# dwofk/fast-depth

Hardware: AMD Instinct MI355X
Metric: frames/sec (224x224) MobileNet-NNConv5dw-skipadd inference forward (higher is better)
Workload: dtype f32; 1 GPU; configs[1]: MobileNet-NNConv5(dw)+skipadd unpruned, batch=32 per GPU, 224x224 fp32 inference forward, inputs resident in HBM; batch_per_gpu=32, global_batch=32, parallelism=frames sharded over 1 GPU(s), no collective, rccl_ranks=0, input_batches_in_rotation=8

## Files before the change

fast-depth_amd/csrc/fd_infer_launch.h:

```cpp
#pragma once
namespace {

template <typename T, int ACT>
int launch_stem(const Layer &L, const float *x, const float *wp, const float *bias, T *y, int B, hipStream_t s)
{
    switch (L.chunk) {
    case 32: FD_LAUNCH((fd_stem3x3s2<T, ACT, 32>), L.grid, dim3(256), L.lds, s, x, wp, bias, y, B, L.in_h, L.in_w, L.d.cout); break;
    case 16: FD_LAUNCH((fd_stem3x3s2<T, ACT, 16>), L.grid, dim3(256), L.lds, s, x, wp, bias, y, B, L.in_h, L.in_w, L.d.cout); break;
    default: FD_LAUNCH((fd_stem3x3s2<T, ACT, 8>), L.grid, dim3(256), L.lds, s, x, wp, bias, y, B, L.in_h, L.in_w, L.d.cout); break;
    }
    return check_launch("fd_stem3x3s2");
}

template <typename T, int K, int S, int MODE, int ACT>
int launch_dw_inst(const Layer &L, const T *in, const T *skip, const float *wp, const float *bias, T *out, hipStream_t s)
{
    if constexpr (!std::is_same<T, float>::value) {
        if (L.dw_n == 8) {
            FD_LAUNCH((fd_dwconv<T, K, S, MODE, ACT, 8>), L.grid, dim3(256), L.lds, s, in, skip, wp, bias, out,
                      L.in_h, L.in_w, L.out_h, L.out_w, L.d.cin, L.cbq, L.th, L.tw, L.tiles_x, L.csplit, L.pstr);
            return check_launch("fd_dwconv");
        }
    }
    FD_LAUNCH((fd_dwconv<T, K, S, MODE, ACT, 4>), L.grid, dim3(256), L.lds, s, in, skip, wp, bias, out,
                       L.in_h, L.in_w, L.out_h, L.out_w, L.d.cin, L.cbq, L.th, L.tw, L.tiles_x, L.csplit, L.pstr);
    return check_launch("fd_dwconv");
}

template <typename T, int ACT>
int launch_dw(const Layer &L, const T *in, const T *skip, const float *wp, const float *bias, T *out, hipStream_t s, const unsigned *wpk = nullptr)
{
    if (L.dw5_cl) {
        if constexpr (!std::is_same<T, float>::value) {
            if (L.dw5_cl == 64)
                FD_LAUNCH((fd_dw5_rows<T, ACT, 64>), L.grid, dim3(FD_DW5R_BLOCK), 0, s, in, skip, wpk, bias, out, L.in_h, L.in_w, L.d.cin, L.dw5_cbs, L.dw5_groups, L.dw5_bh);
            else
                FD_LAUNCH((fd_dw5_rows<T, ACT, 32>), L.grid, dim3(FD_DW5R_BLOCK), 0, s, in, skip, wpk, bias, out, L.in_h, L.in_w, L.d.cin, L.dw5_cbs, L.dw5_groups, L.dw5_bh);
            return check_launch("fd_dw5_rows");
        }
        return fail(FD_ERR_INVALID, "fd_dw5_rows is a 16-bit kernel");
    }
    if (L.dw_rows && L.dw_rows8) {
        if constexpr (!std::is_same<T, float>::value) {
            if (L.d.stride == 1)
                FD_LAUNCH((fd_dw3_rows8<T, 1, ACT>), L.grid, dim3(256), 0, s, in, wp, bias, out, L.in_h, L.in_w, L.out_h, L.out_w, L.d.cin, L.th);
            else
                FD_LAUNCH((fd_dw3_rows8<T, 2, ACT>), L.grid, dim3(256), 0, s, in, wp, bias, out, L.in_h, L.in_w, L.out_h, L.out_w, L.d.cin, L.th);
            return check_launch("fd_dw3_rows8");
        }
    }
    if (L.dw_rows) {
        if (L.d.stride == 1)
            FD_LAUNCH((fd_dw3_rows<T, 1, ACT>), L.grid, dim3(256), 0, s, in, wp, bias, out, L.in_h, L.in_w, L.out_h, L.out_w, L.d.cin, L.th);
        else
            FD_LAUNCH((fd_dw3_rows<T, 2, ACT>), L.grid, dim3(256), 0, s, in, wp, bias, out, L.in_h, L.in_w, L.out_h, L.out_w, L.d.cin, L.th);
        return check_launch("fd_dw3_rows");
    }
    const int key = L.d.ksize * 100 + L.d.stride * 10 + L.mode;
    switch (key) {
    case 310: return launch_dw_inst<T, 3, 1, 0, ACT>(L, in, skip, wp, bias, out, s);
    case 320: return launch_dw_inst<T, 3, 2, 0, ACT>(L, in, skip, wp, bias, out, s);
    case 510: return launch_dw_inst<T, 5, 1, 0, ACT>(L, in, skip, wp, bias, out, s);
    case 511: return launch_dw_inst<T, 5, 1, 1, ACT>(L, in, skip, wp, bias, out, s);
    case 512: return launch_dw_inst<T, 5, 1, 2, ACT>(L, in, skip, wp, bias, out, s);
    case 311: return launch_dw_inst<T, 3, 1, 1, ACT>(L, in, skip, wp, bias, out, s);
    case 312: return launch_dw_inst<T, 3, 1, 2, ACT>(L, in, skip, wp, bias, out, s);
    case 513: return launch_dw_inst<T, 5, 1, 3, ACT>(L, in, skip, wp, bias, out, s);
    }
    return fail(FD_ERR_INVALID, "depthwise k=%d stride=%d mode=%d has no kernel", L.d.ksize, L.d.stride, L.mode);
}

template <int ACT>
int launch_pw(const fd_plan *plan, const Layer &L, const float *A, const float *wp, const float *bias, float *out, long M, hipStream_t s)
{
    const int N = L.d.cout, K = L.d.cin;
    if (L.pw16_tm) {
        fd_dwfuse fz{};
        int fdw = 0;
        if (L.fuse_next_dw >= 0) {
            const Layer &D = plan->layers[L.fuse_next_dw];
            fz.w = reinterpret_cast<const float *>(plan->ws + D.w_off); fz.b = reinterpret_cast<const float *>(plan->ws + D.b_off);
            fz.out = reinterpret_cast<float *>(plan->ws + D.out_off);
            fz.H = L.out_h; fz.W = L.out_w; fz.S = D.d.stride; fz.up = D.d.upsample;
            fz.hi = D.d.act == FD_ACT_RELU6 ? 6.0f : __builtin_inff();
            fz.store_pw = (plan->flags & FD_PLAN_KEEP_ACTIVATIONS) ? 1 : 0;
            fdw = D.d.ksize;
        }
#define FD_PW16_LAUNCH(TMV, FD_) \
        do { (void)hipFuncSetAttribute((const void *)fd_pw_gemm16_f32<TMV, FD_G16_STAGES, ACT, 0, FD_>, hipFuncAttributeMaxDynamicSharedMemorySize, (int)L.lds); \
             FD_LAUNCH((fd_pw_gemm16_f32<TMV, FD_G16_STAGES, ACT, 0, FD_>), L.grid, dim3(512), L.lds, s, A, wp, bias, out, (int)M, N, K, L.w_pitch, L.pw16_stride, L.m_tiles, L.n_tiles, fz, fd_g16_train{}); } while (0)
#define FD_PW16_CASE(TMV) \
    case TMV: if (fdw == 3) FD_PW16_LAUNCH(TMV, 3); else if (fdw == 5) FD_PW16_LAUNCH(TMV, 5); else FD_PW16_LAUNCH(TMV, 0); break;
        switch (L.pw16_tm) {
            FD_PW16_CASE(13)
            FD_PW16_CASE(7)
            FD_PW16_CASE(4)
        default: return fail(FD_ERR_INVALID, "no gemm16 instance for TM=%d", L.pw16_tm);
        }
#undef FD_PW16_CASE
#undef FD_PW16_LAUNCH
        return check_launch("fd_pw_gemm16_f32");
    }
    const int key = L.pw.wgm * 1000 + L.pw.wgn * 100 + L.pw.tm * 10 + L.pw.tn;
#define FD_PW_CASE(a, b, c, d) \
    case a * 1000 + b * 100 + c * 10 + d: \
        if (L.lds > 64 * 1024) (void)hipFuncSetAttribute((const void *)fd_pw_gemm_f32<a, b, c, d, ACT>, hipFuncAttributeMaxDynamicSharedMemorySize, (int)L.lds); \
        FD_LAUNCH((fd_pw_gemm_f32<a, b, c, d, ACT>), L.grid, dim3(256), L.lds, s, A, wp, bias, out, (int)M, N, K, L.w_pitch, L.m_tiles, L.n_tiles); break;
    switch (key) {
        FD_PW_CASE(2, 2, 2, 2)
        FD_PW_CASE(2, 2, 2, 1)
        FD_PW_CASE(2, 2, 1, 2)
        FD_PW_CASE(2, 2, 1, 1)
        FD_PW_CASE(4, 1, 1, 1)
    default: return fail(FD_ERR_INVALID, "no pointwise tile %d", key);
    }
#undef FD_PW_CASE
    return check_launch("fd_pw_gemm_f32");
}



template <int ACT>
int launch_dwpw(const fd_plan *p, const Layer &L, float *out, float *y, hipStream_t s)
// ... 133 lines not shown
```

fast-depth_amd/csrc/fd_kernels_dw5p.h:

```cpp
#pragma once
#include "fd_device.h"

#ifdef FD_EMU
#define FD_INLINE_LAMBDA
#else
#define FD_INLINE_LAMBDA __attribute__((always_inline))
#endif

template <typename T>
__global__ void __launch_bounds__(256)
fd_pack_dw5_pairs(const float *__restrict__ wf, unsigned *__restrict__ wpk, int C)
{
    const int i = blockIdx.x * 256 + threadIdx.x;
    if (i >= 30 * C) return;
    const int c = i % C, q = i / C, ky = q / 6, k = q - ky * 6;
    const float *w = wf + (long)(ky * 5) * C + c;
    const float w0 = w[0], w1 = w[C], w2 = w[2 * C], w3 = w[3 * C], w4 = w[4 * C];
    float a, b;
    switch (k) {
    case 0: a = w0; b = w1; break;
    case 1: a = w2; b = w3; break;
    case 2: a = w4; b = 0.f; break;
    case 3: a = 0.f; b = w0; break;
    case 4: a = w1; b = w2; break;
// ... 92 lines not shown
    auto issue_a = [&](int it) FD_INLINE_LAMBDA {
        const int r = y0 - 2 + 2 * it;
        nv = r >= 0 && r < H;
        if (!nv) return;
        const unsigned ro = (unsigned)r * rowb;
#pragma unroll
        for (int p = 0; p < 4; ++p) { ns[0][2 * p] = fd_buf_ld32(r_skip, so[p], ro); ns[0][2 * p + 1] = fd_buf_ld32(r_skip, so[p], ro + pxb); }
    };
    auto issue_b = [&](int it) FD_INLINE_LAMBDA {
        const int r = y0 - 2 + 2 * it;
        nv_b = r >= 0 && r < H;
        if (!nv_b) return;
        const unsigned ro = (unsigned)(r + 1) * rowb, rl = (unsigned)(r >> 1) * (rowb >> 1);
#pragma unroll
        for (int p = 0; p < 4; ++p) { ns[1][2 * p] = fd_buf_ld32(r_skip, so[p], ro); ns[1][2 * p + 1] = fd_buf_ld32(r_skip, so[p], ro + pxb); nl[p] = fd_buf_ld32(r_low, lo_[p], rl); }
    };

    unsigned win[5][4][2];
#pragma unroll
    for (int a = 0; a < 5; ++a)
#pragma unroll
        for (int p = 0; p < 4; ++p) { win[a][p][0] = 0u; win[a][p][1] = 0u; }

    auto convert = [&](auto SLOT, const unsigned (&raw)[8], bool rv) FD_INLINE_LAMBDA {
        constexpr int slot = decltype(SLOT)::value;
        if (rv) fd_dw5_make_pairs(T{}, raw, nl, win[slot]);
        else {
#pragma unroll
            for (int p = 0; p < 4; ++p) { win[slot][p][0] = 0u; win[slot][p][1] = 0u; }
        }
    };
    auto out_row = [&](auto SB, int y) FD_INLINE_LAMBDA {
        constexpr int sb = decltype(SB)::value;
        float acc[4][2];
#pragma unroll
        for (int ky = 0; ky < 5; ++ky) {
            const unsigned (&R)[4][2] = win[(sb + ky) % 5];
#pragma unroll
            for (int k = 0; k < 3; ++k) {
#pragma unroll
                for (int ch = 0; ch < 2; ++ch) {
                    if (ky == 0 && k == 0) {
                        const float bb = ch ? b1 : b0;
                        acc[0][ch] = fd_dot2_first(T{}, R[k][ch], w[ky][k][ch], bb);
                        acc[1][ch] = fd_dot2_first(T{}, R[k][ch], w[ky][3 + k][ch], bb);
                        acc[2][ch] = fd_dot2_first(T{}, R[k + 1][ch], w[ky][k][ch], bb);
                        acc[3][ch] = fd_dot2_first(T{}, R[k + 1][ch], w[ky][3 + k][ch], bb);
                    } else {
                        fd_dot2_acc(T{}, R[k][ch], w[ky][k][ch], acc[0][ch]);
                        fd_dot2_acc(T{}, R[k][ch], w[ky][3 + k][ch], acc[1][ch]);
                        fd_dot2_acc(T{}, R[k + 1][ch], w[ky][k][ch], acc[2][ch]);
                        fd_dot2_acc(T{}, R[k + 1][ch], w[ky][3 + k][ch], acc[3][ch]);
                    }
                }
            }
        }
        fd_dot2_done(acc);
        if (y < y1) {
#pragma unroll
            for (int j = 0; j < 4; ++j) fd_buf_st32(r_out, oo, (unsigned)y * rowb + (unsigned)j * pxb, fd_dw5_pack_act<T, ACT>(acc[j][0], acc[j][1]));
        }
    };

    const int n_it = (y1 - y0 + 4) >> 1;
    issue_a(0); issue_b(0);
    auto step = [&](auto PH, int it) FD_INLINE_LAMBDA {
        constexpr int ph = decltype(PH)::value;
        const bool more = it + 1 < n_it;
        convert(fd_int<(2 * ph) % 5>{}, ns[0], nv);
        if (more) issue_a(it + 1);
        if (it >= 2) out_row(fd_int<(2 * ph + 1) % 5>{}, y0 - 4 + 2 * it);
        convert(fd_int<(2 * ph + 1) % 5>{}, ns[1], nv_b);
        if (more) issue_b(it + 1);
        if (it >= 2) out_row(fd_int<(2 * ph + 2) % 5>{}, y0 - 3 + 2 * it);
    };
    for (int it0 = 0; it0 < n_it; it0 += 5) {
        step(fd_int<0>{}, it0);
        if (it0 + 1 < n_it) step(fd_int<1>{}, it0 + 1);
        if (it0 + 2 < n_it) step(fd_int<2>{}, it0 + 2);
        if (it0 + 3 < n_it) step(fd_int<3>{}, it0 + 3);
        if (it0 + 4 < n_it) step(fd_int<4>{}, it0 + 4);
    }
}
```

fast-depth_amd/csrc/fd_plan_build.h:

```cpp
#pragma once
namespace {

int plan_layers(fd_plan *p, const fd_layer_desc *layers, size_t *woff_out)
{
    const size_t esz = p->dtype == FD_F32 ? 4 : 2;
    const int n_layers = (int)p->layers.size(), batch = p->B, height = p->H, width = p->W, dtype = p->dtype;
    const uint32_t flags = p->flags, tune = p->tune;
    (void)n_layers; (void)batch; (void)height; (void)width; (void)dtype; (void)flags; (void)tune;
    size_t woff = 0;
    for (int i = 0; i < n_layers; ++i) {
        Layer &L = p->layers[i];
        L.d = layers[i];
        const fd_layer_desc &d = L.d;
#define FD_BAD(...) do { return fail(FD_ERR_INVALID, __VA_ARGS__); } while (0)
        if (d.src >= i || d.skip >= i) FD_BAD("layer %d: src/skip must reference earlier layers", i);
        if (d.act < FD_ACT_NONE || d.act > FD_ACT_RELU6) FD_BAD("layer %d: bad activation", i);
        if (d.cin <= 0 || d.cout <= 0) FD_BAD("layer %d: bad channel counts", i);
        int src_h, src_w, src_c;
        if (d.src < 0) { src_h = height; src_w = width; src_c = 3; }
        else { const Layer &S = p->layers[d.src]; src_h = S.out_h; src_w = S.out_w; src_c = S.d.cout; }
        const bool concat = d.concat != 0;
        if (concat && (d.skip < 0 || d.op != FD_OP_DW || !d.upsample)) FD_BAD("layer %d: concat needs an upsampled depthwise consumer with a skip tensor", i);
        if (concat) {
            L.csplit = src_c;
            if (src_c + p->layers[d.skip].d.cout != d.cin || src_c % 4) FD_BAD("layer %d: concat of %d + %d channels does not give cin %d", i, src_c, p->layers[d.skip].d.cout, d.cin);
        } else if (src_c != d.cin) FD_BAD("layer %d: cin %d != producer channels %d", i, d.cin, src_c);
        L.in_h = d.upsample ? 2 * src_h : src_h;
        L.in_w = d.upsample ? 2 * src_w : src_w;
        if (d.skip >= 0) {
            const Layer &S = p->layers[d.skip];
            if (!d.upsample) FD_BAD("layer %d: skip without upsample is not part of this path", i);
            if (S.out_h != L.in_h || S.out_w != L.in_w || (!concat && S.d.cout != d.cin))
                FD_BAD("layer %d: skip tensor %dx%dx%d does not match input %dx%dx%d", i, S.out_h, S.out_w, S.d.cout, L.in_h, L.in_w, d.cin);
        }
        switch (d.op) {
        case FD_OP_STEM:
            if (d.src != -1 || d.cin != 3 || d.ksize != 3 || d.stride != 2 || d.upsample || d.skip >= 0 || d.cout % 8)
                FD_BAD("layer %d: stem must be 3->8k channels, 3x3 stride 2 on the network input", i);
            L.out_h = L.in_h / 2; L.out_w = L.in_w / 2;
            L.chunk = d.cout % 32 == 0 ? 32 : (d.cout % 16 == 0 ? 16 : 8);
            if (d.cout > 64) FD_BAD("layer %d: the stem supports at most 64 output channels", i);
            {
                const int nrows = 2 * ceil_div(255, L.out_w) + 3;
                L.lds = std::max((size_t)3 * nrows * (L.in_w + 8) * 4, (size_t)4 * 64 * 36 * 4);
            }
            L.grid = dim3(ceil_div((long)L.out_h * L.out_w, 256), batch);
            L.w_bytes = (size_t)27 * d.cout * 4; L.w_elems = (size_t)27 * d.cout;
            break;
        case FD_OP_DW: {
            if (d.src < 0 || d.cin != d.cout || (d.ksize != 3 && d.ksize != 5) || (d.stride != 1 && d.stride != 2) || d.cin % 4)
                FD_BAD("layer %d: depthwise needs cin==cout (multiple of 4), k in {3,5}, stride in {1,2}", i);
            if (d.stride == 2 && (L.in_h % 2 || L.in_w % 2)) FD_BAD("layer %d: stride-2 depthwise on odd input", i);
            L.mode = d.upsample ? (d.skip >= 0 ? (concat ? 3 : 2) : 1) : 0;
            L.out_h = L.in_h / d.stride; L.out_w = L.in_w / d.stride;
            if (d.ksize == 3 && L.mode == 0) {
                L.dw_rows = true;
                L.dw_rows8 = dtype != FD_F32 && d.cin % 8 == 0 && d.stride == 1 && !(flags & FD_PLAN_NO_ROWS8);
                const int gx = ceil_div((long)L.out_w * (d.cin / (L.dw_rows8 ? 8 : 4)), 256);
                int th = L.out_h;
                while (th > 4 && (long)gx * ceil_div(L.out_h, th) * batch < 1024) th = (th + 1) / 2;
                L.th = th;
                L.grid = dim3(gx, ceil_div(L.out_h, th), batch);
                L.lds = 0;
                L.w_bytes = (size_t)9 * d.cin * 4; L.w_elems = (size_t)9 * d.cin;
                break;
            }
            if (dtype != FD_F32 && d.ksize == 5 && d.stride == 1 && L.mode == 2 && d.cin % 8 == 0 && L.out_w % 4 == 0 && L.in_h % 2 == 0 &&
                (double)L.in_h * L.in_w * d.cin * 2.0 < 2147483648.0 && !(tune & FD_TUNE_NO_DW5_ROWS)) {
                const int strips = L.out_w / 4;
                L.dw5_cl = (strips % 2 == 1 && d.cin >= 128) ? 64 : 32;
                const int cblocks = ceil_div(d.cin, 2 * L.dw5_cl);
                L.dw5_cbs = ceil_div(ceil_div(d.cin, cblocks), 8) * 8;
                L.dw5_groups = ceil_div(strips, 64 / L.dw5_cl);
                const int bands = std::max(1, (L.out_h + 7) / 14);
                L.dw5_bh = ceil_div(ceil_div(L.out_h, bands), 2) * 2;
                L.grid = dim3(ceil_div((long)L.dw5_groups * ceil_div(L.out_h, L.dw5_bh), FD_DW5R_BLOCK / 64), cblocks, batch);
                L.lds = 0;
                L.w_elems = (size_t)25 * d.cin;
                L.wpk_off = align_up((size_t)25 * d.cin * 4, 256);
                L.w_bytes = L.wpk_off + (size_t)30 * d.cin * 4;
                break;
            }
            const bool h8_ok = dtype != FD_F32 && d.cin % 8 == 0 && (!concat || L.csplit % 8 == 0) && !(tune & FD_TUNE_NO_DW_H8);
            const bool h8 = h8_ok && ((tune & FD_TUNE_FORCE_DW_H8) || (d.ksize == 5 && d.cin % 64 == 0 && (long)L.out_h * L.out_w >= 56 * 56));
            L.dw_n = h8 ? 8 : 4;
            int cb = d.cin >= 32 ? 32 : (d.cin >= 16 ? 16 : (d.cin >= 8 ? 8 : 4));
            if (h8 && d.cin >= 64 && ceil_div(d.cin, 64) * 64 <= ceil_div(d.cin, 32) * 32) cb = 64;
            L.cbq = ilog2(cb / L.dw_n);
            const int tmax_w = d.stride == 2 ? 8 : 16, tmax_h = d.ksize == 5 ? 7 : 8;
            L.tw = std::min((L.out_w + 3) / 4 * 4, tmax_w);
            L.th = std::min(L.out_h, tmax_h);
            L.tiles_x = ceil_div(L.out_w, L.tw); L.tiles_y = ceil_div(L.out_h, L.th);
            const int th_in = (L.th - 1) * d.stride + d.ksize, tw_in = (L.tw - 1) * d.stride + d.ksize;
            L.pstr = h8 ? 2 * pick_patch_pitch(cb / 2, L.tw, tw_in, d.stride) : pick_patch_pitch(cb, L.tw, tw_in, d.stride);
            L.lds = align_up((size_t)th_in * tw_in * L.pstr * (h8 ? 2 : 4), 16) + ((size_t)d.ksize * d.ksize * cb + cb) * 4;
            L.grid = dim3(L.tiles_x * L.tiles_y, ceil_div(d.cin, cb), batch);
            L.w_bytes = (size_t)d.ksize * d.ksize * d.cin * 4; L.w_elems = (size_t)d.ksize * d.ksize * d.cin;
            break;
        }
        case FD_OP_PW:
            if (d.src < 0 || d.ksize != 1 || d.stride != 1 || d.cin % 4) FD_BAD("layer %d: pointwise needs k=1 stride=1 cin%%4==0", i);
            L.out_h = L.in_h; L.out_w = L.in_w;
            L.w_bytes = (size_t)d.cin * d.cout * 4;
            L.w_elems = (size_t)d.cin * d.cout;
            if (d.cout == 1) {
                if (d.skip >= 0) FD_BAD("layer %d: head with skip is not part of this path", i);
                L.head = true;
                const long npix = (long)batch * (L.in_h >> (d.upsample ? 1 : 0)) * (L.in_w >> (d.upsample ? 1 : 0));
                L.grid = dim3(ceil_div(npix * 8, 256));
            } else {
                if (d.upsample || d.skip >= 0) FD_BAD("layer %d: pointwise after upsample is only supported for the 1-channel head", i);
                const long M = (long)batch * L.out_h * L.out_w;
                if (dtype != FD_F32 && d.cin % 8) FD_BAD("layer %d: 16-bit pointwise needs cin %% 8 == 0", i);
                L.w_pitch = dtype == FD_F32 ? (d.cin + 31) / 32 * 32 : (d.cin + 63) / 64 * 64;
                L.w_bytes = (size_t)d.cout * L.w_pitch * esz;
                L.pw = dtype == FD_F32 ? choose_pw(M, d.cout) : PwCfg{2, 2, 1, 1};
                L.lds = pw_lds_bytes(L.pw);
                if (dtype != FD_F32) L.lds = (size_t)std::min(FD_H16_STAGES, ceil_div(d.cin, 64)) * 128 * 128;
                L.m_tiles = ceil_div(M, L.pw.wgm * L.pw.tm * 32);
                L.n_tiles = ceil_div(d.cout, L.pw.wgn * L.pw.tn * 32);
                L.grid = dim3((unsigned)((L.m_tiles + 7) / 8 * 8 * L.n_tiles));
                if ((dtype == FD_F32 || (tune & FD_TUNE_FORCE_GEMM16)) && !(flags & FD_PLAN_NO_GEMM16)) {
                    const Pw16Cfg c16 = choose_pw16(M, d.cout, d.cin, (tune & FD_TUNE_FORCE_GEMM16) != 0);
                    if (c16.tm) {
                        L.pw16_tm = c16.tm; L.pw16_stride = c16.stride;
                        L.lds = (size_t)(dtype == FD_F32 ? FD_G16_STAGES : 4) * (c16.tm * 16 + 64) * 32 * 4;
                        L.m_tiles = ceil_div(M, c16.stride); L.n_tiles = ceil_div(d.cout, 64);
                        L.grid = dim3((unsigned)((L.m_tiles + 7) / 8 * 8 * L.n_tiles));
                    }
                }
            }
            break;
        default: FD_BAD("layer %d: unknown op %d", i, d.op);
        }
        if (L.lds > 160 * 1024) FD_BAD("layer %d: LDS request %zu exceeds 160 KiB", i, L.lds);
        if ((long)L.in_h * L.in_w >= (1L << 24) || d.cin >= (1 << 24) || d.cout >= (1 << 24) || (double)L.in_h * L.in_w * std::max(d.cin, d.cout) >= 4294967296.0)
            FD_BAD("layer %d: a %dx%d map with %d channels exceeds the kernels' 32-bit within-image addressing", i, L.in_h, L.in_w, std::max(d.cin, d.cout));
        L.w_off = woff; woff += align_up(L.w_bytes, 256);
        if (L.dw5_cl) L.wpk_off += L.w_off;
        L.b_off = woff; woff += align_up((size_t)d.cout * 4, 256);
        L.out_bytes = align_up((size_t)batch * L.out_h * L.out_w * d.cout * esz, 256);
        L.pw_packed_t = (d.op == FD_OP_PW && !L.head && dtype != FD_F32);
    }
    Layer &last = p->layers.back();
    if (last.d.cout != 1 || last.out_h != height || last.out_w != width)
        FD_BAD("the last layer must produce the [B,1,%d,%d] network output (got %dx%dx%d)", height, width, last.out_h, last.out_w, last.d.cout);
#undef FD_BAD
    last.to_output = true;
    p->weights_bytes = woff;

    *woff_out = woff;
    return FD_OK;
}

void plan_fuse_epilogues(fd_plan *p)
{
    const int n_layers = (int)p->layers.size(), batch = p->B, height = p->H, width = p->W, dtype = p->dtype;
    const uint32_t flags = p->flags, tune = p->tune;
    (void)n_layers; (void)batch; (void)height; (void)width; (void)dtype; (void)flags; (void)tune;
    if (!(flags & FD_PLAN_NO_EPILOGUE_FUSION)) {
        std::vector<int> readers(n_layers, 0);
        for (int i = 0; i < n_layers; ++i) {
            if (p->layers[i].d.src >= 0) ++readers[p->layers[i].d.src];
// ... 107 lines not shown
            if (p->layers[i].d.src >= 0) ++rd[p->layers[i].d.src];
            if (p->layers[i].d.skip >= 0) ++rd[p->layers[i].d.skip];
        }
        for (int i = 0; i + 1 < n_layers; ++i) {
            Layer &Pw = p->layers[i], &H = p->layers[i + 1];
            if (Pw.d.op != FD_OP_PW || Pw.head || Pw.pw16_tm || Pw.dwpw || Pw.fuse_next_dw >= 0 || Pw.skipped || Pw.fused_into >= 0 || Pw.to_output) continue;
            if (!H.head || H.d.src != i || H.d.skip >= 0 || rd[i] != 1 || H.d.cin != Pw.d.cout || Pw.d.cout > 32 || Pw.d.cout % 8 || Pw.n_tiles != 1) continue;
            Pw.fuse_head = i + 1; H.fused_into = i;
        }
    }

}

void plan_arena(fd_plan *p, size_t woff)
{
    const int n_layers = (int)p->layers.size(), batch = p->B, height = p->H, width = p->W, dtype = p->dtype;
    const uint32_t flags = p->flags, tune = p->tune;
    (void)n_layers; (void)batch; (void)height; (void)width; (void)dtype; (void)flags; (void)tune;
    std::vector<int> last_use(n_layers, -1);
    for (int i = 0; i < n_layers; ++i) {
        if (p->layers[i].d.src >= 0) last_use[p->layers[i].d.src] = i;
        if (p->layers[i].d.skip >= 0) last_use[p->layers[i].d.skip] = i;
        if (p->layers[i].fused_dw >= 0) {
            const fd_layer_desc &dd = p->layers[p->layers[i].fused_dw].d;
            last_use[dd.src] = i;
            if (dd.skip >= 0) last_use[dd.skip] = i;
        }
    }
    FreeList fl;
    std::vector<char> released(n_layers, 0);
    for (int i = 0; i < n_layers; ++i) {
        Layer &L = p->layers[i];
        if (!(flags & FD_PLAN_KEEP_ACTIVATIONS))
            for (int j = 0; j < i; ++j)
                if (!released[j] && last_use[j] >= 0 && last_use[j] <= i - 1 && !p->layers[j].to_output && !p->layers[j].skipped) {
                    fl.release(p->layers[j].out_off - woff, p->layers[j].out_bytes);
                    released[j] = 1;
                }
        if (L.to_output || L.skipped) continue;
        if (L.fused_into >= 0) continue;
        L.out_off = woff + fl.alloc(L.out_bytes);
        if (L.fuse_next_dw >= 0) p->layers[L.fuse_next_dw].out_off = woff + fl.alloc(p->layers[L.fuse_next_dw].out_bytes);
    }
    p->ws_bytes = woff + fl.top;

}

void plan_describe(fd_plan *p)
{
    const int n_layers = (int)p->layers.size(), batch = p->B, height = p->H, width = p->W, dtype = p->dtype;
    const uint32_t flags = p->flags, tune = p->tune;
    (void)n_layers; (void)batch; (void)height; (void)width; (void)dtype; (void)flags; (void)tune;
    const size_t esz = dtype == FD_F32 ? 4 : 2;
    for (int i = 0; i < n_layers; ++i) {
        Layer &L = p->layers[i];
        const fd_layer_desc &d = L.d;
        const int c_src = L.csplit ? L.csplit : d.cin, c_skip = L.csplit ? d.cin - L.csplit : d.cin;
        const double src_elems = (double)batch * (d.upsample ? (L.in_h / 2) * (L.in_w / 2) : L.in_h * L.in_w) * c_src;
        const double skip_elems = d.skip >= 0 ? (double)batch * L.in_h * L.in_w * c_skip : 0.0;
        const double out_elems = (double)batch * L.out_h * L.out_w * d.cout;
        const double in_esz = d.src < 0 ? 4.0 : (double)esz, out_esz = L.to_output ? 4.0 : (double)esz;
        L.alg_bytes = (src_elems + skip_elems) * in_esz + out_elems * out_esz + (double)L.w_elems * (L.pw_packed_t ? esz : 4) + 2.0 * d.cout * 4;
        p->alg_bytes += L.alg_bytes;
        const double taps = d.op == FD_OP_STEM ? 27.0 : (d.op == FD_OP_DW ? (double)d.ksize * d.ksize : (double)d.cin);
        const double mac_px = L.head && d.upsample ? (double)L.out_h * L.out_w : (double)L.out_h * L.out_w;
        L.alg_flops = 2.0 * batch * mac_px * d.cout * taps;
        p->alg_flops += L.alg_flops;
        char buf[256];
        if (L.skipped)
            snprintf(buf, sizeof buf, "(fused into layer %d)", i + 1);
        else if (L.fused_into >= 0 && L.head)
            snprintf(buf, sizeof buf, "(pointwise head evaluated on the accumulators of layer %d's %s kernel)", L.fused_into, p->layers[L.fused_into].dwpw ? "dwpw" : "pw_gemm");
        else if (L.fused_into >= 0)
            snprintf(buf, sizeof buf, "(dw k%d s%d%s evaluated in the epilogue of layer %d's pw_gemm16)", d.ksize, d.stride, d.upsample ? " on up2" : "", L.fused_into);
        else if (L.dwpw)
            snprintf(buf, sizeof buf, "dwpw<dw k%d s%d mode%d + pw> persistent, 4 producer + 4 consumer waves; tile %dx%d px x all %d channels, C=%d in %d chunks, weights in LDS, grid=%u lds=%zu%s", p->layers[L.fused_dw].d.ksize,
                     p->layers[L.fused_dw].d.stride, p->layers[L.fused_dw].mode, L.dp_th, 1 << L.dp_tw, d.cout, d.cin, d.cin / 32, L.grid.x, L.lds,
                     L.fuse_head >= 0 ? " + the 32->1 head on the accumulators" : "");
        else if (d.op == FD_OP_STEM)
            snprintf(buf, sizeof buf, "stem3x3s2<mfma 32x32x2, LDS-staged rows, 256 px per workgroup> grid=%ux%u lds=%zu", L.grid.x, L.grid.y, L.lds);
        else if (d.op == FD_OP_DW && L.dw5_cl)
            snprintf(buf, sizeof buf, "dw5_rows<k5 s1 mode2, pixel pairs + dot2, %d channel lanes per strip> bands of %d rows, %d strip groups, %d channels per block, grid=%ux%ux%u, no LDS",
                     L.dw5_cl, L.dw5_bh, L.dw5_groups, L.dw5_cbs, L.grid.x, L.grid.y, L.grid.z);
        else if (d.op == FD_OP_DW && L.dw_rows)
            snprintf(buf, sizeof buf, "dw3_rows%s<s%d> rows/item %d grid=%ux%ux%u", L.dw_rows8 ? "8" : "", d.stride, L.th, L.grid.x, L.grid.y, L.grid.z);
        else if (d.op == FD_OP_DW)
            snprintf(buf, sizeof buf, "dwconv<k%d s%d mode%d> tile %dx%dx%d pitch %d grid=%ux%ux%u lds=%zu, %d channels per work-item", d.ksize, d.stride, L.mode,
                     L.th, L.tw, L.dw_n << L.cbq, L.pstr, L.grid.x, L.grid.y, L.grid.z, L.lds, L.dw_n);
        else if (L.head)
            snprintf(buf, sizeof buf, "head_pw1 up=%d grid=%u", d.upsample, L.grid.x);
        else
            if (L.pw16_tm)
                snprintf(buf, sizeof buf, "pw_gemm16<TM=%d: %dx64 tile, stride %d> M=%ld N=%d K=%d tiles=%dx%d (%.2f per CU) lds=%zu", L.pw16_tm, L.pw16_tm * 16, L.pw16_stride,
                         (long)batch * L.out_h * L.out_w, d.cout, d.cin, L.m_tiles, L.n_tiles, L.m_tiles * L.n_tiles / 256.0, L.lds),
                L.fuse_next_dw >= 0 ? (void)snprintf(buf + strlen(buf), sizeof buf - strlen(buf), " + fused dw k%d of layer %d", p->layers[L.fuse_next_dw].d.ksize, L.fuse_next_dw) : (void)0;
            else
            snprintf(buf, sizeof buf, "pw_gemm<%dx%d> M=%ld N=%d K=%d tiles=%dx%d lds=%zu", L.pw.wgm * L.pw.tm * 32,
                     L.pw.wgn * L.pw.tn * 32, (long)batch * L.out_h * L.out_w, d.cout, d.cin, L.m_tiles, L.n_tiles, L.lds),
            (L.fuse_head >= 0 && !L.dwpw) ? (void)snprintf(buf + strlen(buf), sizeof buf - strlen(buf), " + the %d->1 head on its output tile", d.cout) : (void)0;
        L.info = buf;
        const char *tn = dtype == FD_F32 ? "float" : (dtype == FD_F16 ? "_Float16" : "fd_bf16");
        if (L.skipped || L.fused_into >= 0) buf[0] = 0;
        else if (L.dwpw) snprintf(buf, sizeof buf, "fd_dwpw_f32<%d, %d, %d, %d, %d, %d, %d, %d, 0>", p->layers[L.fused_dw].d.ksize, p->layers[L.fused_dw].d.stride, p->layers[L.fused_dw].mode, d.act, L.dp_wm, L.dp_nt, L.dp_nld, L.fuse_head >= 0 ? 1 : 0);
        else if (d.op == FD_OP_STEM) snprintf(buf, sizeof buf, "fd_stem3x3s2<%s, %d, %d>", tn, d.act, L.chunk);
        else if (d.op == FD_OP_DW && L.dw5_cl) snprintf(buf, sizeof buf, "fd_dw5_rows<%s, %d, %d>", tn, d.act, L.dw5_cl);
        else if (d.op == FD_OP_DW && L.dw_rows) snprintf(buf, sizeof buf, "fd_dw3_rows%s<%s, %d, %d>", L.dw_rows8 ? "8" : "", tn, d.stride, d.act);
        else if (d.op == FD_OP_DW) snprintf(buf, sizeof buf, "fd_dwconv<%s, %d, %d, %d, %d, %d>", tn, d.ksize, d.stride, L.mode, d.act, L.dw_n);
        else if (L.head) snprintf(buf, sizeof buf, "fd_head_pw1<%s, %d>", tn, d.act);
        else if (L.pw16_tm && dtype != FD_F32) snprintf(buf, sizeof buf, "fd_pw_gemm16_h16<%s, %d, 4, %d, %d, 1>", tn, L.pw16_tm, d.act, L.fuse_next_dw >= 0 ? p->layers[L.fuse_next_dw].d.ksize : 0);
        else if (L.pw16_tm) snprintf(buf, sizeof buf, "fd_pw_gemm16_f32<%d, %d, %d, 0, %d, 0>", L.pw16_tm, FD_G16_STAGES, d.act, L.fuse_next_dw >= 0 ? p->layers[L.fuse_next_dw].d.ksize : 0);
        else if (dtype == FD_F32) snprintf(buf, sizeof buf, "fd_pw_gemm_f32<%d, %d, %d, %d, %d>", L.pw.wgm, L.pw.wgn, L.pw.tm, L.pw.tn, d.act);
        else if (L.fuse_head >= 0) snprintf(buf, sizeof buf, "fd_pw_gemm_head_h16<%s, %d>", tn, d.act);
        else snprintf(buf, sizeof buf, "fd_pw_gemm_h16<%s, %d>", tn, d.act);
        L.sym = buf;
    }
}

}
```

fast-depth_amd/csrc/fd_plan_select.h:

```cpp
#pragma once
#ifndef FD_G16_STAGES
#define FD_G16_STAGES 4
#endif
namespace {

int pick_patch_pitch(int cb, int tw, int tw_in, int stride, int strip = 4)
{
    static const int grp[4][16] = {{0, 1, 2, 3, 12, 13, 14, 15, 20, 21, 22, 23, 24, 25, 26, 27}, {4, 5, 6, 7, 8, 9, 10, 11, 16, 17, 18, 19, 28, 29, 30, 31},
                                   {32, 33, 34, 35, 44, 45, 46, 47, 52, 53, 54, 55, 56, 57, 58, 59}, {36, 37, 38, 39, 40, 41, 42, 43, 48, 49, 50, 51, 60, 61, 62, 63}};
    const int lanes_c = cb / 4, tws = std::max(1, tw / strip);
    int cbq = 0; while ((1 << cbq) < lanes_c) ++cbq;
    int best = cb + 4; long best_cycles = -1;
    for (int pitch = cb + 4; pitch <= cb + 36; pitch += 4) {
        long cycles = 0;
        for (int wave = 0; wave < 4; ++wave)
            for (int g = 0; g < 4; ++g) {
                int first_addr[64][4], n_addr[64];
                for (int b = 0; b < 64; ++b) n_addr[b] = 0;
                for (int k = 0; k < 16; ++k) {
                    const int tid = wave * 64 + grp[g][k], c4 = tid & (lanes_c - 1), pt = tid >> cbq;
                    const int oy = pt / tws, ox = (pt - oy * tws) * strip;
                    const int addr = ((oy * stride) * tw_in + ox * stride) * pitch + c4 * 4;
                    for (int dw = 0; dw < 4; ++dw) {
                        const int b = (addr + dw) & 63;
                        bool seen = false;
                        for (int q = 0; q < n_addr[b] && q < 4; ++q) seen |= first_addr[b][q] == addr;
                        if (!seen) { if (n_addr[b] < 4) first_addr[b][n_addr[b]] = addr; ++n_addr[b]; }
                    }
                }
                int worst = 1;
                for (int b = 0; b < 64; ++b) worst = std::max(worst, n_addr[b]);
                cycles += worst;
            }
        if (best_cycles < 0 || cycles < best_cycles) { best_cycles = cycles; best = pitch; }
        if (cycles == 16) break;
    }
    return best;
}

struct PwCfg { int wgm, wgn, tm, tn; };

struct Layer {
    fd_layer_desc d;
    int in_h = 0, in_w = 0;
    int out_h = 0, out_w = 0;
    size_t out_off = 0, out_bytes = 0;
    size_t w_off = 0, w_bytes = 0, b_off = 0;
    size_t w_elems = 0;
    bool to_output = false;
    bool head = false;
    bool pw_packed_t = false;
    int cbq = 0, th = 0, tw = 0, tiles_x = 0, tiles_y = 0, mode = 0, pstr = 0;
    int dw_n = 4;
    int dw5_cl = 0, dw5_cbs = 0, dw5_groups = 0, dw5_bh = 0;
    size_t wpk_off = 0;
    int csplit = 0;
    bool skipped = false;
    int fuse_next_dw = -1;
    int fused_into = -1;
    int fused_dw = -1;
    int fuse_head = -1;
    bool dwpw = false;
    int dp_th = 0, dp_tw = 0 , dp_tiles_x = 0, dp_wm = 0, dp_nt = 0, dp_nld = 0, dp_xcd = 0;
    bool dw_rows = false;
    bool dw_rows8 = false;
    int chunk = 0;
    PwCfg pw{};
    int m_tiles = 0, n_tiles = 0, w_pitch = 0;
    int pw16_tm = 0, pw16_stride = 0;
    size_t lds = 0;
    dim3 grid;
    std::string info, sym;
    double alg_bytes = 0, alg_flops = 0;
};

}

struct fd_plan {
    std::vector<Layer> layers;
    int B = 0, H = 0, W = 0, dtype = 0;
    uint32_t flags = 0, tune = 0;
    size_t ws_bytes = 0, weights_bytes = 0;
    unsigned char *ws = nullptr;
    bool packed = false;
    double alg_bytes = 0, alg_flops = 0;
};

namespace {

struct FreeList {
    std::vector<std::pair<size_t, size_t>> blocks;
    size_t top = 0;
    size_t alloc(size_t bytes)
    {
        for (size_t i = 0; i < blocks.size(); ++i)
            if (blocks[i].second >= bytes) {
                size_t off = blocks[i].first;
                blocks[i].first += bytes;
                blocks[i].second -= bytes;
                if (blocks[i].second == 0) blocks.erase(blocks.begin() + i);
                return off;
            }
        if (!blocks.empty() && blocks.back().first + blocks.back().second == top) {
            size_t off = blocks.back().first;
            top = off + bytes;
            blocks.pop_back();
            return off;
        }
        size_t off = top;
        top += bytes;
        return off;
    }
    void release(size_t off, size_t bytes)
    {
        auto it = std::lower_bound(blocks.begin(), blocks.end(), std::make_pair(off, (size_t)0));
        it = blocks.insert(it, {off, bytes});
        if (it + 1 != blocks.end() && it->first + it->second == (it + 1)->first) { it->second += (it + 1)->second; blocks.erase(it + 1); }
        if (it != blocks.begin() && (it - 1)->first + (it - 1)->second == it->first) { (it - 1)->second += it->second; blocks.erase(it); }
    }
};

PwCfg choose_pw(long M, int N)
{
    const PwCfg c128x128{2, 2, 2, 2}, c128x64{2, 2, 2, 1}, c64x128{2, 2, 1, 2}, c64x64{2, 2, 1, 1}, c128x32{4, 1, 1, 1};
    if (N <= 32) return c128x32;
    auto blocks = [&](const PwCfg &c) { return (long)ceil_div(M, c.wgm * c.tm * 32) * ceil_div(N, c.wgn * c.tn * 32); };
    auto waste = [&](const PwCfg &c) { int bn = c.wgn * c.tn * 32; return (double)(ceil_div(N, bn) * bn) / N; };
    (void)blocks; (void)waste; (void)c128x128;
    if (M > 4096 && M <= 16384 && N >= 512) return c64x128;
    if (M > 16384 && M <= 32768 && N > 32 && N <= 128) return c128x64;
    return c64x64;
}

struct Pw16Cfg { int tm = 0, stride = 0; double score = 0; };
Pw16Cfg choose_pw16(long M, int N, int K, bool force)
{
    Pw16Cfg best;
// ... 25 lines not shown
```

fast-depth_amd/csrc/fd_tuning.h:

```cpp
#pragma once
#include <stdint.h>

#define FD_TUNE_WGRAD_TILE_ROWS 1u
#define FD_TUNE_FORCE_GEMM16 2u
#define FD_TUNE_FORCE_EPILOGUE_FUSION 4u
#define FD_TUNE_FORCE_UNIT_FUSION 8u
#define FD_TUNE_NO_PW_PAIRING 16u
#define FD_TUNE_PW_PAIR_TN2 32u
#define FD_TUNE_DW_BWD1 64u
#define FD_TUNE_DW_BWD_PAIR 128u
#define FD_TUNE_DW_SMALL_TILES 256u
#define FD_TUNE_DW_PITCH4 512u
#define FD_TUNE_DW_PITCH8 1024u
#define FD_TUNE_DW_WGRAD_TH4 2048u
#define FD_TUNE_DW_NO_ROWS 4096u
#define FD_TUNE_DW_FORCE_ROWS 8192u
#define FD_TUNE_DW_TH8 16384u
#define FD_TUNE_DW_CB16 32768u
#define FD_TUNE_NO_DW_H8 65536u
#define FD_TUNE_FORCE_DW_H8 131072u
#define FD_TUNE_NO_CONSUMER_FINALIZE 262144u
#define FD_TUNE_DW_BWD_FINALIZE 524288u
#define FD_TUNE_NO_DW5_ROWS 1048576u
#define FD_TUNE_ALL 2097151u

#ifdef __cplusplus
extern "C" {
#endif
void fd_tuning_next(uint32_t mask);
struct fd_train_plan;
int fd_train_plan_lds_rounding(const struct fd_train_plan *plan, int32_t layer);
int fd_train_plan_unit_kernels(const struct fd_train_plan *plan, int32_t layer);
struct fd_comm;
void fd_comm_elide_collectives(struct fd_comm *comm, int32_t on);
int fd_comm_bind_library(const char *path);
#ifdef __cplusplus
}
#endif
```

fast-depth_amd/fastdepth_hip/capi.py:

```python
import ctypes
import os

HERE = os.path.dirname(os.path.abspath(__file__))
DEFAULT_LIB = os.path.join(HERE, "libfastdepth_hip.so")

FD_F32, FD_F16, FD_BF16 = 0, 1, 2


class _DtypeMap(dict):
    def __missing__(self, key):
        import torch
        m = {torch.float32: FD_F32, torch.float16: FD_F16, torch.bfloat16: FD_BF16}
        self.update(m)
        return m[key]


DTYPE_OF = _DtypeMap()
FD_OP_STEM, FD_OP_DW, FD_OP_PW = 0, 1, 2
FD_ACT_NONE, FD_ACT_RELU, FD_ACT_RELU6 = 0, 1, 2
FD_PLAN_KEEP_ACTIVATIONS = 1
FD_PLAN_NO_GEMM16 = 64
FD_PLAN_NO_ROWS8 = 256
FD_PLAN_NO_EPILOGUE_FUSION = 512
FD_PLAN_NO_UNIT_FUSION = 1024
FD_PLAN_NO_BWD_PAIRING = 4096
_TUNE_SHIFT = 32
FD_TUNE_WGRAD_TILE_ROWS = 1 << _TUNE_SHIFT
FD_TUNE_FORCE_GEMM16 = 2 << _TUNE_SHIFT
FD_TUNE_FORCE_EPILOGUE_FUSION = 4 << _TUNE_SHIFT
FD_TUNE_FORCE_UNIT_FUSION = 8 << _TUNE_SHIFT
FD_TUNE_NO_PW_PAIRING = 16 << _TUNE_SHIFT
FD_TUNE_PW_PAIR_TN2 = 32 << _TUNE_SHIFT
FD_TUNE_DW_BWD1 = 64 << _TUNE_SHIFT
FD_TUNE_DW_BWD_PAIR = 128 << _TUNE_SHIFT
FD_TUNE_DW_SMALL_TILES = 256 << _TUNE_SHIFT
FD_TUNE_DW_PITCH4 = 512 << _TUNE_SHIFT
FD_TUNE_DW_PITCH8 = 1024 << _TUNE_SHIFT
FD_TUNE_DW_WGRAD_TH4 = 2048 << _TUNE_SHIFT
FD_TUNE_DW_NO_ROWS = 4096 << _TUNE_SHIFT
FD_TUNE_DW_FORCE_ROWS = 8192 << _TUNE_SHIFT
FD_TUNE_DW_TH8 = 16384 << _TUNE_SHIFT
FD_TUNE_DW_CB16 = 32768 << _TUNE_SHIFT
FD_TUNE_NO_DW_H8 = 65536 << _TUNE_SHIFT
FD_TUNE_FORCE_DW_H8 = 131072 << _TUNE_SHIFT
FD_TUNE_NO_CONSUMER_FINALIZE = 262144 << _TUNE_SHIFT
FD_TUNE_DW_BWD_FINALIZE = 524288 << _TUNE_SHIFT
FD_TUNE_NO_DW5_ROWS = 1048576 << _TUNE_SHIFT


def create_plan(lib, train, descs, n, batch, height, width, fd_dtype, flags, handle_ref):
    tuning = int(flags) >> _TUNE_SHIFT
    lib.fd_tuning_next(tuning)
    fn = lib.fd_train_plan_create if train else lib.fd_plan_create
    return fn(descs, n, batch, height, width, fd_dtype, int(flags) & 0xFFFFFFFF, handle_ref)


def parse_flags(text):
    v = 0
    for tok in str(text).replace(",", "|").split("|"):
        tok = tok.strip()
        if not tok:
            continue
        g = globals()
        if "FD_PLAN_" + tok in g:
            v |= g["FD_PLAN_" + tok]
        elif "FD_TUNE_" + tok in g:
            v |= g["FD_TUNE_" + tok]
        else:
            v |= int(tok, 0)
    return v


class LayerDesc(ctypes.Structure):
    _fields_ = [(n, ctypes.c_int32) for n in
                ("op", "cin", "cout", "ksize", "stride", "act", "src", "upsample", "skip", "concat")]


class LayerParams(ctypes.Structure):
    _fields_ = [(n, ctypes.c_void_p) for n in ("conv_weight", "bn_weight", "bn_bias", "bn_mean", "bn_var", "bn_num_batches_tracked")]


class LayerGrads(ctypes.Structure):
    _fields_ = [(n, ctypes.c_void_p) for n in ("conv_weight", "bn_weight", "bn_bias")]


class GradBucket(ctypes.Structure):
    _fields_ = [("from_layer", ctypes.c_int32), ("to_layer", ctypes.c_int32), ("grad", ctypes.c_void_p), ("numel", ctypes.c_int64), ("grad16", ctypes.c_void_p)]


class TraceRecord(ctypes.Structure):
    _fields_ = [("kernel", ctypes.c_char_p), ("layer", ctypes.c_int32), ("ms", ctypes.c_float)]


class SgdTensor(ctypes.Structure):
    _fields_ = [("param", ctypes.c_void_p), ("grad", ctypes.c_void_p), ("momentum_buf", ctypes.c_void_p), ("numel", ctypes.c_int64)]


class AugParams(ctypes.Structure):
    _fields_ = [("s", ctypes.c_double), ("angle", ctypes.c_double), ("brightness", ctypes.c_float), ("contrast", ctypes.c_float),
                ("saturation", ctypes.c_float), ("flip", ctypes.c_int32), ("order", ctypes.c_int32 * 3), ("reserved", ctypes.c_int32)]


class FastDepthError(RuntimeError):
    pass


def load(path=None):
    path = path or DEFAULT_LIB
    if not os.path.exists(path):
        raise FastDepthError("HIP extension not built: %s is missing (run `python fast-depth_amd/build.py`)" % path)
    lib = ctypes.CDLL(path)
    vp, i32, u32 = ctypes.c_void_p, ctypes.c_int32, ctypes.c_uint32
    lib.fd_plan_create.argtypes = [ctypes.POINTER(LayerDesc), i32, i32, i32, i32, i32, u32, ctypes.POINTER(vp)]
    lib.fd_plan_create.restype = ctypes.c_int
    lib.fd_tuning_next.argtypes = [u32]
    lib.fd_tuning_next.restype = None
    lib.fd_plan_destroy.argtypes = [vp]
    lib.fd_plan_destroy.restype = None
    lib.fd_plan_workspace_bytes.argtypes = [vp]
    lib.fd_plan_workspace_bytes.restype = ctypes.c_size_t
    lib.fd_plan_bind_workspace.argtypes = [vp, vp, ctypes.c_size_t]
    lib.fd_plan_bind_workspace.restype = ctypes.c_int
    lib.fd_plan_pack_weights.argtypes = [vp, ctypes.POINTER(LayerParams), i32, ctypes.c_float, vp]
    lib.fd_plan_pack_weights.restype = ctypes.c_int
    lib.fd_forward.argtypes = [vp, vp, vp, vp]
    lib.fd_forward.restype = ctypes.c_int
    lib.fd_forward_timed.argtypes = [vp, vp, vp, vp, ctypes.POINTER(ctypes.c_float), i32]
    lib.fd_forward_timed.restype = ctypes.c_int
    lib.fd_layer_output.argtypes = [vp, i32, ctypes.POINTER(vp)] + [ctypes.POINTER(i32)] * 4
    lib.fd_layer_output.restype = ctypes.c_int
# ... 106 lines not shown
```

Measured before the change: 42440 frames/s.

## Add fp32 register-window 5x5 depthwise row kernel for skip-add decoder layers

Adds an fp32 kernel for 5x5 stride-1 mode-2 depthwise layers, which fuse nearest upsampling of the low-res input with the skip add. Each lane handles one channel across four columns and keeps a rotating five-row register window, so loads for the next rows are issued while the current row is computed. It uses buffer loads and no LDS, and the plan picks a band height from the batch and grid size. The aim is to replace the generic tiled fp32 dwconv path for the decoder layers. It costs more register pressure and fixes waves per EU at 4.

```diff
diff --git a/fast-depth_amd/csrc/fd_infer_launch.h b/fast-depth_amd/csrc/fd_infer_launch.h
--- a/fast-depth_amd/csrc/fd_infer_launch.h
+++ b/fast-depth_amd/csrc/fd_infer_launch.h
@@ -39,6 +39,13 @@
             return check_launch("fd_dw5_rows");
         }
         return fail(FD_ERR_INVALID, "fd_dw5_rows is a 16-bit kernel");
+    }
+    if (L.dw5_f32) {
+        if constexpr (std::is_same<T, float>::value) {
+            FD_LAUNCH((fd_dw5_rows_f32<ACT>), L.grid, dim3(FD_DW5R_BLOCK), 0, s, in, skip, wp, bias, out, L.in_h, L.in_w, L.d.cin, L.dw5_groups, L.dw5_bh);
+            return check_launch("fd_dw5_rows_f32");
+        }
+        return fail(FD_ERR_INVALID, "fd_dw5_rows_f32 is an fp32 kernel");
     }
     if (L.dw_rows && L.dw_rows8) {
         if constexpr (!std::is_same<T, float>::value) {
diff --git a/fast-depth_amd/csrc/fd_kernels_dw5p.h b/fast-depth_amd/csrc/fd_kernels_dw5p.h
--- a/fast-depth_amd/csrc/fd_kernels_dw5p.h
+++ b/fast-depth_amd/csrc/fd_kernels_dw5p.h
@@ -198,3 +198,122 @@
         if (it0 + 4 < n_it) step(fd_int<4>{}, it0 + 4);
     }
 }
+
+#ifdef FD_EMU
+inline float fd_dw5_mac(float a, float b, float c) { return c + a * b; }
+#else
+__device__ __forceinline__ float fd_dw5_mac(float a, float b, float c) { return __builtin_fmaf(a, b, c); }
+#endif
+#ifndef FD_DW5R32_BAND
+#define FD_DW5R32_BAND 0
+#endif
+#ifndef FD_DW5R32_WAVES
+#define FD_DW5R32_WAVES 4
+#endif
+#ifdef FD_EMU
+#define FD_DW5R32_ATTR
+#else
+#define FD_DW5R32_ATTR __attribute__((amdgpu_waves_per_eu(FD_DW5R32_WAVES, FD_DW5R32_WAVES)))
+#endif
+
+template <int ACT>
+__global__ void __launch_bounds__(FD_DW5R_BLOCK) FD_DW5R32_ATTR
+fd_dw5_rows_f32(const float *__restrict__ low, const float *__restrict__ skip, const float *__restrict__ wp, const float *__restrict__ bias,
+                float *__restrict__ out, int H, int W, int C, int groups_x, int bh)
+{
+    const fd_blk3 blk = fd_xcd_image_map();
+    const int item = blk.x * (FD_DW5R_BLOCK / 64) + FD_UNIFORM((int)(threadIdx.x >> 6));
+    const int band = item / groups_x, sg = item - band * groups_x;
+    if (band * bh >= H) return;
+    const int n = blk.z, c = blk.y * 64 + (int)(threadIdx.x & 63), xs = 4 * sg;
+    const int y0 = band * bh, y1 = y0 + bh < H ? y0 + bh : H;
+    if (c >= C) return;
+    const int Hs = H >> 1, Ws = W >> 1;
+
+    float w[25];
+#pragma unroll
+    for (int t = 0; t < 25; ++t) w[t] = wp[(long)t * C + c];
+    const float b0 = bias[c];
+
+    unsigned so[4], lo_[4];
+#pragma unroll
+    for (int p = 0; p < 4; ++p) {
+        const int x = xs - 2 + 2 * p;
+        const bool in = x >= 0 && x < W;
+        so[p] = in ? (fd_mul24((unsigned)x, (unsigned)C) + (unsigned)c) * 4u : FD_BUF_OOB;
+        lo_[p] = in ? (fd_mul24((unsigned)(x >> 1), (unsigned)C) + (unsigned)c) * 4u : FD_BUF_OOB;
+    }
+    const unsigned rowb = fd_mul24((unsigned)W, (unsigned)C) * 4u, pxb = (unsigned)C * 4u;
+    const fd_bufrsrc r_skip = fd_make_rsrc(skip + (long)n * H * W * C, (unsigned)H * rowb);
+    const fd_bufrsrc r_low = fd_make_rsrc(low + (long)n * Hs * Ws * C, (unsigned)Hs * (rowb >> 1));
+    const fd_bufrsrc r_out = fd_make_rsrc(out + (long)n * H * W * C, (unsigned)H * rowb);
+
+    unsigned ns[2][8], nl[4];
+    bool nv = false, nv_b = false;
+    auto issue_a = [&](int it) FD_INLINE_LAMBDA {
+        const int r = y0 - 2 + 2 * it;
+        nv = r >= 0 && r < H;
+        if (!nv) return;
+        const unsigned ro = (unsigned)r * rowb;
+#pragma unroll
+        for (int p = 0; p < 4; ++p) { ns[0][2 * p] = fd_buf_ld32(r_skip, so[p], ro); ns[0][2 * p + 1] = fd_buf_ld32(r_skip, so[p], ro + pxb); }
+    };
+    auto issue_b = [&](int it) FD_INLINE_LAMBDA {
+        const int r = y0 - 2 + 2 * it;
+        nv_b = r >= 0 && r < H;
+        if (!nv_b) return;
+        const unsigned ro = (unsigned)(r + 1) * rowb, rl = (unsigned)(r >> 1) * (rowb >> 1);
+#pragma unroll
+        for (int p = 0; p < 4; ++p) { ns[1][2 * p] = fd_buf_ld32(r_skip, so[p], ro); ns[1][2 * p + 1] = fd_buf_ld32(r_skip, so[p], ro + pxb); nl[p] = fd_buf_ld32(r_low, lo_[p], rl); }
+    };
+
+    float win[5][8];
+#pragma unroll
+    for (int a = 0; a < 5; ++a)
+#pragma unroll
+        for (int i = 0; i < 8; ++i) win[a][i] = 0.0f;
+
+    auto convert = [&](auto SLOT, const unsigned (&raw)[8], bool rv) FD_INLINE_LAMBDA {
+        constexpr int slot = decltype(SLOT)::value;
+#pragma unroll
+        for (int i = 0; i < 8; ++i)
+            win[slot][i] = rv ? __builtin_bit_cast(float, nl[i >> 1]) + __builtin_bit_cast(float, raw[i]) : 0.0f;
+    };
+    auto out_row = [&](auto SB, int y) FD_INLINE_LAMBDA {
+        constexpr int sb = decltype(SB)::value;
+        float acc[4] = {b0, b0, b0, b0};
+#pragma unroll
+        for (int ky = 0; ky < 5; ++ky) {
+            const float (&R)[8] = win[(sb + ky) % 5];
+#pragma unroll
+            for (int kx = 0; kx < 5; ++kx)
+#pragma unroll
+                for (int j = 0; j < 4; ++j) acc[j] = fd_dw5_mac(R[j + kx], w[ky * 5 + kx], acc[j]);
+        }
+        if (y < y1) {
+#pragma unroll
+            for (int j = 0; j < 4; ++j)
+                fd_buf_st32(r_out, so[1 + (j >> 1)], (unsigned)y * rowb + (unsigned)(j & 1) * pxb, __builtin_bit_cast(unsigned, fd_act<ACT>(acc[j])));
+        }
+    };
+
+    const int n_it = (y1 - y0 + 4) >> 1;
+    issue_a(0); issue_b(0);
+    auto step = [&](auto PH, int it) FD_INLINE_LAMBDA {
+        constexpr int ph = decltype(PH)::value;
+        const bool more = it + 1 < n_it;
+        convert(fd_int<(2 * ph) % 5>{}, ns[0], nv);
+        if (more) issue_a(it + 1);
+        if (it >= 2) out_row(fd_int<(2 * ph + 1) % 5>{}, y0 - 4 + 2 * it);
+        convert(fd_int<(2 * ph + 1) % 5>{}, ns[1], nv_b);
+        if (more) issue_b(it + 1);
+        if (it >= 2) out_row(fd_int<(2 * ph + 2) % 5>{}, y0 - 3 + 2 * it);
+    };
+    for (int it0 = 0; it0 < n_it; it0 += 5) {
+        step(fd_int<0>{}, it0);
+        if (it0 + 1 < n_it) step(fd_int<1>{}, it0 + 1);
+        if (it0 + 2 < n_it) step(fd_int<2>{}, it0 + 2);
+        if (it0 + 3 < n_it) step(fd_int<3>{}, it0 + 3);
+        if (it0 + 4 < n_it) step(fd_int<4>{}, it0 + 4);
+    }
+}
diff --git a/fast-depth_amd/csrc/fd_plan_build.h b/fast-depth_amd/csrc/fd_plan_build.h
--- a/fast-depth_amd/csrc/fd_plan_build.h
+++ b/fast-depth_amd/csrc/fd_plan_build.h
@@ -79,6 +79,20 @@
                 L.w_elems = (size_t)25 * d.cin;
                 L.wpk_off = align_up((size_t)25 * d.cin * 4, 256);
                 L.w_bytes = L.wpk_off + (size_t)30 * d.cin * 4;
+                break;
+            }
+            if (dtype == FD_F32 && d.ksize == 5 && d.stride == 1 && L.mode == 2 && L.in_h % 2 == 0 && L.in_w % 2 == 0 &&
+                (double)L.in_h * L.in_w * d.cin * 4.0 < 2147483648.0 && !(tune & FD_TUNE_NO_DW5_ROWS_F32)) {
+                L.dw5_f32 = true;
+                L.dw5_groups = ceil_div(L.out_w, 4);
+                const long per_band = (long)L.dw5_groups * ceil_div(d.cin, 64) * batch;
+                int bands = std::max(1, (L.out_h + 7) / 14);
+                if (FD_DW5R32_BAND > 0) bands = std::max(1, (L.out_h + FD_DW5R32_BAND / 2) / FD_DW5R32_BAND);
+                else if (per_band <= 4096) bands = (int)std::max<long>(1, std::min<long>(4096 / per_band, L.out_h / 6));
+                L.dw5_bh = ceil_div(ceil_div(L.out_h, bands), 2) * 2;
+                L.grid = dim3(ceil_div((long)L.dw5_groups * ceil_div(L.out_h, L.dw5_bh), FD_DW5R_BLOCK / 64), ceil_div(d.cin, 64), batch);
+                L.lds = 0;
+                L.w_bytes = (size_t)25 * d.cin * 4; L.w_elems = (size_t)25 * d.cin;
                 break;
             }
             const bool h8_ok = dtype != FD_F32 && d.cin % 8 == 0 && (!concat || L.csplit % 8 == 0) && !(tune & FD_TUNE_NO_DW_H8);
@@ -352,6 +366,9 @@
         else if (d.op == FD_OP_DW && L.dw5_cl)
             snprintf(buf, sizeof buf, "dw5_rows<k5 s1 mode2, pixel pairs + dot2, %d channel lanes per strip> bands of %d rows, %d strip groups, %d channels per block, grid=%ux%ux%u, no LDS",
                      L.dw5_cl, L.dw5_bh, L.dw5_groups, L.dw5_cbs, L.grid.x, L.grid.y, L.grid.z);
+        else if (d.op == FD_OP_DW && L.dw5_f32)
+            snprintf(buf, sizeof buf, "dw5_rows_f32<k5 s1 mode2, 1 channel x 4 columns per lane, register window> bands of %d rows, %d strips, grid=%ux%ux%u, no LDS",
+                     L.dw5_bh, L.dw5_groups, L.grid.x, L.grid.y, L.grid.z);
         else if (d.op == FD_OP_DW && L.dw_rows)
             snprintf(buf, sizeof buf, "dw3_rows%s<s%d> rows/item %d grid=%ux%ux%u", L.dw_rows8 ? "8" : "", d.stride, L.th, L.grid.x, L.grid.y, L.grid.z);
         else if (d.op == FD_OP_DW)
@@ -374,6 +391,7 @@
         else if (L.dwpw) snprintf(buf, sizeof buf, "fd_dwpw_f32<%d, %d, %d, %d, %d, %d, %d, %d, 0>", p->layers[L.fused_dw].d.ksize, p->layers[L.fused_dw].d.stride, p->layers[L.fused_dw].mode, d.act, L.dp_wm, L.dp_nt, L.dp_nld, L.fuse_head >= 0 ? 1 : 0);
         else if (d.op == FD_OP_STEM) snprintf(buf, sizeof buf, "fd_stem3x3s2<%s, %d, %d>", tn, d.act, L.chunk);
         else if (d.op == FD_OP_DW && L.dw5_cl) snprintf(buf, sizeof buf, "fd_dw5_rows<%s, %d, %d>", tn, d.act, L.dw5_cl);
+        else if (d.op == FD_OP_DW && L.dw5_f32) snprintf(buf, sizeof buf, "fd_dw5_rows_f32<%d>", d.act);
         else if (d.op == FD_OP_DW && L.dw_rows) snprintf(buf, sizeof buf, "fd_dw3_rows%s<%s, %d, %d>", L.dw_rows8 ? "8" : "", tn, d.stride, d.act);
         else if (d.op == FD_OP_DW) snprintf(buf, sizeof buf, "fd_dwconv<%s, %d, %d, %d, %d, %d>", tn, d.ksize, d.stride, L.mode, d.act, L.dw_n);
         else if (L.head) snprintf(buf, sizeof buf, "fd_head_pw1<%s, %d>", tn, d.act);
diff --git a/fast-depth_amd/csrc/fd_plan_select.h b/fast-depth_amd/csrc/fd_plan_select.h
--- a/fast-depth_amd/csrc/fd_plan_select.h
+++ b/fast-depth_amd/csrc/fd_plan_select.h
@@ -53,6 +53,7 @@
     int cbq = 0, th = 0, tw = 0, tiles_x = 0, tiles_y = 0, mode = 0, pstr = 0;
     int dw_n = 4;
     int dw5_cl = 0, dw5_cbs = 0, dw5_groups = 0, dw5_bh = 0;
+    bool dw5_f32 = false;
     size_t wpk_off = 0;
     int csplit = 0;
     bool skipped = false;
diff --git a/fast-depth_amd/csrc/fd_tuning.h b/fast-depth_amd/csrc/fd_tuning.h
--- a/fast-depth_amd/csrc/fd_tuning.h
+++ b/fast-depth_amd/csrc/fd_tuning.h
@@ -22,7 +22,8 @@
 #define FD_TUNE_NO_CONSUMER_FINALIZE 262144u
 #define FD_TUNE_DW_BWD_FINALIZE 524288u
 #define FD_TUNE_NO_DW5_ROWS 1048576u
-#define FD_TUNE_ALL 2097151u
+#define FD_TUNE_NO_DW5_ROWS_F32 2097152u
+#define FD_TUNE_ALL 4194303u
 
 #ifdef __cplusplus
 extern "C" {
diff --git a/fast-depth_amd/fastdepth_hip/capi.py b/fast-depth_amd/fastdepth_hip/capi.py
--- a/fast-depth_amd/fastdepth_hip/capi.py
+++ b/fast-depth_amd/fastdepth_hip/capi.py
@@ -46,6 +46,7 @@
 FD_TUNE_NO_CONSUMER_FINALIZE = 262144 << _TUNE_SHIFT
 FD_TUNE_DW_BWD_FINALIZE = 524288 << _TUNE_SHIFT
 FD_TUNE_NO_DW5_ROWS = 1048576 << _TUNE_SHIFT
+FD_TUNE_NO_DW5_ROWS_F32 = 2097152 << _TUNE_SHIFT
 
 
 def create_plan(lib, train, descs, n, batch, height, width, fd_dtype, flags, handle_ref):
```

Result: no change. 42520 frames/s (median of 2 runs) (+0.2%).
